# Soltanilara/av-aloha

Hardware: AMD Instinct MI355X
Metric: env-steps/sec (whole node) at 4096 parallel envs, SlotInsertion-3Arms (higher is better)
Workload: dtype f32

## Files before the change

av_aloha_amd/csrc/avsim_api.hip:

```cpp
#include <hip/hip_runtime.h>

#include <cmath>
#include <cstdarg>
#include <cstdio>
#include <cstdlib>
#include <cstring>
#include <memory>
#include <string>
#include <thread>
#include <vector>

#include "../../include/avsim.h"
#include "avsim_episode.hip.h"
#include "avsim_ik.hip.h"
#include "avsim_jpeg.hip.h"
#include "avsim_model.h"
#include "avsim_phys.hip.h"
#include "avsim_render.hip.h"
#include "avsim_vis.hip.h"

using namespace avs;

static thread_local std::string g_create_error;

// ... 352 lines not shown
        h->nq = b.scalar("nq"); h->nv = b.scalar("nv"); h->nu = b.scalar("nu");
        h->task_id = b.scalar("task_id"); h->num_arms = b.scalar("num_arms");
        h->nj = h->num_arms == 3 ? 21 : 14;
        static const int mx[5] = {4, 4, 5, 3, 4};
        h->max_reward = mx[h->task_id];
        h->obj_qadr = b.i("objects_qposadr");
        h->nobj = (int)h->obj_qadr.size();
        h->obs_qadr = b.i("obs_qposadr");
        h->qpos_home = b.f("qpos_home");
        h->ctrl_home = b.f("ctrl_home");
        fill_ik(b, h->ik);
        std::string perr;
        if (!h->phys.init(b, num_envs, h->f64, perr)) { g_create_error = perr; return AVSIM_EMODEL; }
        h->render.build(b, num_envs);
        h->vis.keep_instances(b);
    } catch (const std::exception& ex) {
        g_create_error = std::string("avsim_create: ") + ex.what();
        return AVSIM_EMODEL;
    }
    e = hipStreamCreateWithFlags(&h->stream, hipStreamNonBlocking);
    if (e != hipSuccess) { g_create_error = std::string("hipStreamCreate: ") + hipGetErrorString(e); return AVSIM_EHIP; }
    h->own_stream = true;
    for (auto& ev : h->ev) (void)hipEventCreate(&ev);
    size_t N = num_envs, r = h->rsz();
    if (hipMalloc(&h->d_qpos, N * h->nq * r) != hipSuccess || hipMalloc(&h->d_qvel, N * h->nv * r) != hipSuccess ||
        hipMalloc(&h->d_ctrl, N * h->nu * r) != hipSuccess || hipMalloc(&h->d_warm, N * h->nv * r) != hipSuccess ||
        hipMalloc((void**)&h->d_latch, N * sizeof(int)) != hipSuccess) {
        g_create_error = "avsim_create: hipMalloc of the state arrays failed";
        avsim_destroy(h.release());
        return AVSIM_EHIP;
// ... 751 lines not shown
```

av_aloha_amd/csrc/avsim_phys.hip.h:

```cpp
#pragma once
#include <hip/hip_runtime.h>

#include <string>
#include <vector>

#include "avsim_collide.hip.h"
#include "avsim_math.hip.h"
#include "avsim_model.h"

namespace avs {

enum { J_FREE = 0, J_BALL = 1, J_SLIDE = 2, J_HINGE = 3 };
enum { R_EQ = 0, R_FLOSS = 1, R_LIMIT = 2, R_CONTACT = 3 };
constexpr int TREE_W = 8;
constexpr int ROW_W = 2 * TREE_W;
constexpr int ROW_S = ROW_W;
constexpr int RS_S = 9;
constexpr int CAND_MAX = 256;
constexpr int PROF_W = 26;
constexpr int ANC_MAX = 64;
constexpr int NEAR_MAX = 512;

template <typename real>
struct DevModel {
    int nq, nv, nu, nbody, njnt, ngeom, npair, ntree, neq, nfloss, nlimited, nment, task_id, nj, msize;
    real timestep, gravity[3], impratio, grip_lo, grip_hi;
    int noslip_iters;
    int noslip_trees;
    int qcqp_tridiag;
    int newton_early_exit;
    int newton_component;
    int noslip_per_tree;
    int solver, newton_iters;
    real newton_tol, nscale;
    real ls_tolerance;
    int ls_iterations;
// ... 55 lines not shown
    GLB_PTR(const int) eq_qpos1;
    GLB_PTR(const int) eq_qpos2;
    GLB_PTR(const real) eq_polycoef;
    GLB_PTR(const real) eq_solref;
    GLB_PTR(const real) eq_solimp;
    GLB_PTR(const real) qpos0;
    GLB_PTR(const real) qpos_home;
    int nobj;
    GLB_PTR(const int) obj_qadr;
    const double* obj_reset;
    GLB_PTR(const int) geom_type;
    GLB_PTR(const int) geom_body;
    GLB_PTR(const int) geom_hull;
    GLB_PTR(const int) geom_class;
    GLB_PTR(const int) geom_static;
    GLB_PTR(const real) geom_pos;
    GLB_PTR(const real) geom_mat;
    GLB_PTR(const real) geom_size;
    GLB_PTR(const real) geom_cpos;
    GLB_PTR(const real) geom_rbound;
    GLB_PTR(const real) geom_xpos0;
    GLB_PTR(const real) geom_xmat0;
    GLB_PTR(const real) geom_cen0;
    GLB_PTR(const real) geom_aabb0;
    GLB_PTR(const real) geom_lbox;
    GLB_PTR(const real) hull_vert;
    int hull_ovf;
    GLB_PTR(const int) pair_geom;
    GLB_PTR(const int) pair_condim;
    GLB_PTR(const real) pair_friction;
    GLB_PTR(const real) pair_solref;
    GLB_PTR(const real) pair_solimp;
    GLB_PTR(const real) pair_margin;
    GLB_PTR(const real) pair_gap;
    real* rJ_glob;
    real* rB_glob;
    real* gA_glob;
    int* near_glob;
    int* cand_glob;
    real* gref_glob;
    real* bxo_glob;
    GLB_PTR(const int) obs_qposadr;
    GLB_PTR(const real) obs_offset;
    GLB_PTR(const real) obs_scale;
};

struct MOff {
    int nreal, nint;
    int body_parent;
// ... 1930 lines not shown
        {
            const int t = lane >> 3, i = lane & 7;
            const bool mine = t < ka->m.ntree && i < tree_dofnum_()[t];
            const int k = mine ? tree_dofadr_()[t] + i : 0;
            const real x = tree_solve(r + ka->lay.L, mine ? as[k] : real(0));
            GSYNC();
            if (mine) as[k] = x;
        }
        GSYNC();
    }

    __device__ void load_shape(int g, Shape<real>& s) {
        LDS_BASES();
        real *xpos = r + ka->lay.xpos, *xmat = r + ka->lay.xmat, *gcen = r + ka->lay.gcen;
        s.type = geom_type_()[g];
        for (int k = 0; k < 3; k++) s.size[k] = ka->m.geom_size[3 * g + k];
        s.hull = ka->m.hull_vert;
        s.hbase = ka->m.geom_hull[2 * g];
        s.hR = ka->m.geom_hull[2 * g + 1];
        s.hovf = ka->m.hull_ovf;
        s.nh = 0;
        for (int k = 0; k < 3; k++) { s.lc[k] = ka->m.geom_lbox[6 * g + k]; s.lh[k] = ka->m.geom_lbox[6 * g + 3 + k]; }
        if (geom_static_()[g]) {
            for (int k = 0; k < 3; k++) { s.pos[k] = ka->m.geom_xpos0[3 * g + k]; s.center[k] = ka->m.geom_cen0[3 * g + k]; }
            for (int k = 0; k < 9; k++) s.mat[k] = ka->m.geom_xmat0[9 * g + k];
        } else {
            int b = geom_body_()[g];
            real gp[3] = {ka->m.geom_pos[3 * g], ka->m.geom_pos[3 * g + 1], ka->m.geom_pos[3 * g + 2]}, t3[3];
            mulmat(xmat + 9 * b, gp, t3);
            for (int k = 0; k < 3; k++) { s.pos[k] = xpos[3 * b + k] + t3[k]; s.center[k] = gcen[3 * g + k]; }
            const real* Rb = xmat + 9 * b;
            GLB_PTR(const real) Rg = ka->m.geom_mat + 9 * g;
            for (int i = 0; i < 3; i++)
                for (int j = 0; j < 3; j++) s.mat[3 * i + j] = Rb[3 * i] * Rg[j] + Rb[3 * i + 1] * Rg[3 + j] + Rb[3 * i + 2] * Rg[6 + j];
        }
    }

    __device__ AVS_OUTLINE_0 static void multi_perturb(KPtr<real> ka_, real* r_, int* i_, int lane_, int grp_, const real* lr_, const int* li_, int env_,
                                                                   int pga, int pgb, int src, int pert) {
        Env e(ka_, r_, i_, lane_, grp_, lr_, li_);
        e.env = env_;
        LDS_PTR(real) os = (LDS_PTR(real))(e.r + e.ka->lay.scr + SLOT_W * src);
        const real p0[3] = {os[SLOT_P], os[SLOT_P + 1], os[SLOT_P + 2]}, n0[3] = {os[SLOT_N], os[SLOT_N + 1], os[SLOT_N + 2]};
        Shape<real> a, b;
        e.load_shape(pga, a);
        e.load_shape(pgb, b);
        real dk = real(1e30), pk[3] = {0, 0, 0};
        if (!mpr_perturbed(a, b, p0, n0, pert, &dk, pk)) dk = real(1e30);
        os[1 + pert] = dk;
        for (int c = 0; c < 3; c++) os[SLOT_P + 3 * (1 + pert) + c] = pk[c];
    }

    __device__ AVS_OUTLINE void collide() {
        Env e(*this);
        e.collide_i();
        diverged = e.diverged; nit_sum = e.nit_sum; nit_max = e.nit_max; t_broad = e.t_broad; t_narrow = e.t_narrow;
    }
    __device__ __attribute__((always_inline)) void collide_i() {
        PHASE_BEGIN();
        real* gcen = r + ka->lay.gcen;
        int* misc = ii + ka->lay.misc;
        GLB_PTR(int) cand = cand_();
        int ncand = 0;
        long long tb0 = __builtin_readcyclecounter();
        const real skin = real(0.03);
        GLB_PTR(real) gref = gref_();
        GLB_PTR(int) nearl = near_();
        auto pair_hit = [&](int p, real pad) -> bool {
            int g1 = ka->m.pair_geom[2 * p], g2 = ka->m.pair_geom[2 * p + 1];
            bool s1 = geom_static_()[g1], s2 = geom_static_()[g2];
            real mg = ka->m.pair_margin[p] + pad;
            if (s1 || s2) {
                int gs = s1 ? g1 : g2, gd = s1 ? g2 : g1;
                real rd = geom_rbound_()[gd] + mg, d2 = 0;
                for (int k = 0; k < 3; k++) {
                    real c = gcen[3 * gd + k], lo = ka->m.geom_aabb0[6 * gs + k], hi = ka->m.geom_aabb0[6 * gs + 3 + k];
                    real e = c < lo ? lo - c : (c > hi ? c - hi : real(0));
                    d2 += e * e;
                }
                return !(d2 > rd * rd);
            }
            real d[3], rr = geom_rbound_()[g1] + geom_rbound_()[g2] + mg;
            sub3(gcen + 3 * g2, gcen + 3 * g1, d);
            return !(dot3(d, d) > rr * rr);
        };
        bool moved = false;
        if (misc[7]) {
            for (int g = lane; g < ka->m.ngeom; g += G)
                if (!geom_static_()[g]) {
                    const real d[3] = {gcen[3 * g] - gref[3 * g], gcen[3 * g + 1] - gref[3 * g + 1], gcen[3 * g + 2] - gref[3 * g + 2]};
                    moved |= dot3(d, d) > real(0.25) * skin * skin;
                }
        }
        bool rebuild = !misc[7] || __any(moved);
        int nnear = misc[6];
        if (rebuild) {
            nnear = 0;
            for (int base = 0; base < ka->m.npair; base += G) {
                int p = base + lane;
                bool hit = p < ka->m.npair && pair_hit(p, skin);
                int tot, rk = group_rank<G>(hit, grp, lane, &tot);
                if (hit && nnear + rk < NEAR_MAX) nearl[nnear + rk] = p;
                nnear += tot;
            }
            for (int i = lane; i < 3 * ka->m.ngeom; i += G) gref[i] = gcen[i];
            if (lane == 0) { misc[6] = nnear < NEAR_MAX ? nnear : NEAR_MAX; misc[7] = nnear <= NEAR_MAX; if (nnear > NEAR_MAX) misc[2] |= 8; }
            GSYNC();
        }
        if (nnear <= NEAR_MAX) {
            for (int base = 0; base < nnear; base += G) {
                int i = base + lane, p = i < nnear ? nearl[i] : 0;
                bool hit = i < nnear && pair_hit(p, real(0));
                int tot, rk = group_rank<G>(hit, grp, lane, &tot);
                if (hit && ncand + rk < CAND_MAX) cand[ncand + rk] = p;
                if (ncand + tot > CAND_MAX && lane == 0) misc[2] |= 4;
                ncand = ncand + tot < CAND_MAX ? ncand + tot : CAND_MAX;
            }
        } else {
            for (int base = 0; base < ka->m.npair; base += G) {
                int p = base + lane;
                bool hit = p < ka->m.npair && pair_hit(p, real(0));
                int tot, rk = group_rank<G>(hit, grp, lane, &tot);
                if (hit && ncand + rk < CAND_MAX) cand[ncand + rk] = p;
                if (ncand + tot > CAND_MAX && lane == 0) misc[2] |= 4;
                ncand = ncand + tot < CAND_MAX ? ncand + tot : CAND_MAX;
            }
        }
        if (lane == 0) misc[3] = ncand;
        GSYNC();
        long long tb1 = __builtin_readcyclecounter();
        t_broad += tb1 - tb0;
        real *cdist = r + ka->lay.cdist, *cpos = r + ka->lay.cpos, *cnrm = r + ka->lay.cnrm;
        int* cpair = ii + ka->lay.cpair;
        int ncon = 0, ovf = 0;
        int* mlist = ii + ka->lay.cand;
        GLB_PTR(real) bxo = bxo_();
        for (int base = 0; base < ncand; base += G) {
            const int ci = base + lane;
            int n = 0, p = 0, nn = 0;
            LDS_PTR(real) scr = (LDS_PTR(real))(r + ka->lay.scr + SLOT_W * lane);
            const bool valid = ci < ncand;
            if (valid) p = cand[ci];
            const int ga = ka->m.pair_geom[2 * p], gb = ka->m.pair_geom[2 * p + 1];
            const int tya = geom_type_()[ga], tyb = geom_type_()[gb];
            const bool isbox = valid && tya == G_BOX && tyb == G_BOX;
            const long long tn0_ = profiling ? __builtin_readcyclecounter() : 0;
            {
                bool boxlive = false;
                if (isbox) {
                    Shape<real> a, b;
                    load_shape(ga, a);
                    load_shape(gb, b);
                    boxlive = !boxes_separated(a, b);
                }
                int nbox, rk = group_rank<G>(boxlive, grp, lane, &nbox);
                const int row = lane >> 4;
                for (int b0 = 0; b0 < nbox; b0 += 4) {
                    int src = 0;
// ... 47 lines not shown
                            const real dk = scr[k];
                            const real pk[3] = {scr[SLOT_P + 3 * k], scr[SLOT_P + 3 * k + 1], scr[SLOT_P + 3 * k + 2]};
                            if (dk < real(1e29) && multiccd_distinct(pk, scr + SLOT_P, kept, tol)) {
                                scr[kept] = dk;
                                for (int c = 0; c < 3; c++) scr[SLOT_P + 3 * kept + c] = pk[c];
                                kept++;
                            }
                        }
                        nn = kept;
                    }
                }
            }
            int keepmask = 0;
            GLB_PTR(const real) ov = bxo + BOX_OVF_W * lane;
            if (valid) {
                real mg = ka->m.pair_margin[p];
                for (int k = 0; k < nn; k++)
                    if ((isbox && k >= BOX_SLOTC ? ov[4 * (k - BOX_SLOTC)] : scr[k]) < mg) { keepmask |= 1 << k; n++; }
            }
            int off = 0, tot = 0;
            for (int j = 1; j <= BOX_MAXC; j++) {
                int tj, rj = group_rank<G>(n >= j, grp, lane, &tj);
                if (tj == 0) break;
                off += rj;
                tot += tj;
            }
            int w = 0;
            for (int k = 0; k < BOX_MAXC; k++)
                if ((keepmask >> k) & 1) {
                    int c = ncon + off + w;
                    w++;
// ... 53 lines not shown
            }
            int t1, t2, r1 = group_rank<G>(lo, grp, lane, &t1), r2 = group_rank<G>(hi, grp, lane, &t2);
            int pos = nefc + r1 + r2;
            if (lo && pos < ka->lay.maxefc) rmeta[pos] = R_LIMIT | (j << 2) | (0 << 12);
            if (hi && pos + lo < ka->lay.maxefc) rmeta[pos + lo] = R_LIMIT | (j << 2) | (1 << 12);
            nefc += t1 + t2;
        }
        int ovf = 0;
        if (nefc > ka->lay.maxefc) { nefc = ka->lay.maxefc; ovf = 1; }
        if (lane == 0) misc[4] = nefc;
        const int nlead0 = nefc;
        int cend = nefc;
        for (int base = 0; base < ncon; base += G) {
            int c = base + lane, dim = 0;
            if (c < ncon) {
                int p = cpair[c];
                if (cdist[c] < ka->m.pair_margin[p] - ka->m.pair_gap[p]) dim = ka->m.pair_condim[p];
            }
            int off = 0, tot = 0;
            for (int j = 1; j <= 6; j++) {
                int tj, rj = group_rank<G>(dim >= j, grp, lane, &tj);
                off += rj;
                tot += tj;
            }
            int myend = 0;
            if (c < ncon) {
                int first = nefc + off;
                if (dim > 0 && first + dim <= ka->lay.maxefc) {
                    cefc[c] = first | (dim << 16);
                    myend = first + dim;
                    for (int s = 0; s < dim; s++) rmeta[first + s] = R_CONTACT | (c << 2) | (s << 12) | (dim << 20);
                } else {
// ... 51 lines not shown
                j1 = d - tree_dofadr_()[tA]; v1 = 1;
                for (int k = 0; k < 2; k++) solref[k] = ka->m.dof_solref[2 * d + k];
                for (int k = 0; k < 5; k++) solimp[k] = ka->m.dof_solimp[5 * d + k];
            } else if (LEAD && type == R_LIMIT) {
                int j = id, d = jnt_dofadr_()[j];
                real q = qpos[jnt_qposadr_()[j]];
                tA = dof_tree_()[d];
                pos = sub == 0 ? q - jnt_range_()[2 * j] : jnt_range_()[2 * j + 1] - q;
                margin = jnt_margin_()[j];
                diag0 = dof_invweight0_()[d];
                j1 = d - tree_dofadr_()[tA]; v1 = sub == 0 ? real(1) : real(-1);
                for (int k = 0; k < 2; k++) solref[k] = ka->m.jnt_solref[2 * j + k];
                for (int k = 0; k < 5; k++) solimp[k] = ka->m.jnt_solimp[5 * j + k];
            } else if (!LEAD) {
                int c = id, p = cpair[c];
                int g1 = ka->m.pair_geom[2 * p], g2 = ka->m.pair_geom[2 * p + 1], b1 = geom_body_()[g1], b2 = geom_body_()[g2];
                int t1 = body_tree_()[b1], t2 = body_tree_()[b2];
                tA = t1 >= 0 ? t1 : t2;
                tB = (t1 >= 0 && t2 >= 0 && t2 != t1) ? t2 : -1;
                real n[3] = {cnrm[3 * c], cnrm[3 * c + 1], cnrm[3 * c + 2]}, t1v[3], t2v[3], cp[3] = {cpos[3 * c], cpos[3 * c + 1], cpos[3 * c + 2]};
                make_frame(n, t1v, t2v);
                const int sm = sub % 3;
                real ax[3];
#pragma unroll
                for (int q = 0; q < 3; q++) ax[q] = sm == 0 ? n[q] : (sm == 1 ? t1v[q] : t2v[q]);
                const bool rot = sub >= 3;
                real cx[3], Wa[3], Wl[3];
                cross3(cp, ax, cx);
#pragma unroll
                for (int q = 0; q < 3; q++) { Wa[q] = rot ? ax[q] : cx[q]; Wl[q] = rot ? real(0) : ax[q]; }
                const int mA = (t1 == tA ? bmask[b1] : 0), pA = (t2 == tA ? bmask[b2] : 0);
// ... 2 lines not shown
#pragma unroll
                for (int k = 0; k < TREE_W; k++) {
                    const real* ca = cdofp + 6 * (aA + k < nvm ? aA + k : nvm);
                    const real ea = Wa[0] * ca[0] + Wa[1] * ca[1] + Wa[2] * ca[2] + Wl[0] * ca[3] + Wl[1] * ca[4] + Wl[2] * ca[5];
                    J[k] = real(((pA >> k) & 1) - ((mA >> k) & 1)) * ea;
                }
                if (tB >= 0) {
#pragma unroll
                    for (int k = 0; k < TREE_W; k++) {
                        const real* cb = cdofp + 6 * (aB + k < nvm ? aB + k : nvm);
                        const real eb = Wa[0] * cb[0] + Wa[1] * cb[1] + Wa[2] * cb[2] + Wl[0] * cb[3] + Wl[1] * cb[4] + Wl[2] * cb[5];
                        J[TREE_W + k] = real(((pB >> k) & 1) - ((mB >> k) & 1)) * eb;
                    }
                }
                pos = sub == 0 ? cdist[c] : real(0);
                margin = ka->m.pair_margin[p] - ka->m.pair_gap[p];
                diag0 = body_invweight0_()[2 * b1] + body_invweight0_()[2 * b2];
                for (int k = 0; k < 2; k++) solref[k] = ka->m.pair_solref[2 * p + k];
                for (int k = 0; k < 5; k++) solimp[k] = ka->m.pair_solimp[5 * p + k];
            }
            (void)valid;
            const int j2c = j2 >= 0 ? j2 : (j1 >= 0 ? j1 : 0), j1c = j1 >= 0 ? j1 : 0;
            const real v2c = j2 >= 0 ? v2 : real(0);
            if (LEAD) {
#pragma unroll
                for (int k = 0; k < TREE_W; k++) J[k] += (k == j1 ? v1 : real(0)) + (k == j2 ? v2 : real(0));
            }
            real dmax = tclamp(solimp[1], real(0.0001), real(0.9999));
            real tc = tmax(solref[0], 2 * ka->m.timestep), dr = solref[1];
            real K = real(1) / tmax(real(1e-15), dmax * dmax * tc * tc * dr * dr), Bd = real(2) / tmax(real(1e-15), dmax * tc);
            real imp, R;
            const real imp_row = impedance(solimp, (!LEAD && sub > 0) ? cdist[id] : pos, margin);
            if (!LEAD && sub > 0) {
                int c = id, p = cpair[c];
                real imp0 = imp_row;
                real R0 = tmax(real(1e-15), (1 - imp0) * diag0 / imp0);
                real R1 = R0 / tmax(real(1e-15), ka->m.impratio);
                real mu0 = ka->m.pair_friction[5 * p], mur = ka->m.pair_friction[5 * p + sub - 1];
                R = sub == 1 ? R1 : R1 * mu0 * mu0 / tmax(real(1e-15), mur * mur);
                imp = imp0;
                K = 0;
                floss = mur;
            } else {
                imp = imp_row;
                R = tmax(real(1e-15), (1 - imp) * diag0 / imp);
            }
            real vel = 0;
            if (LEAD) {
                const int a0 = tadr[tA];
                vel = v1 * qvel[a0 + j1c] + v2c * qvel[a0 + j2c];
            } else {
                const int a0 = tadr[tA], b0 = tadr[tB >= 0 ? tB : tA];
#pragma unroll
// ... 89 lines not shown
        for (int i = lane; i < nlead0; i += G) fill(i, BoolTag<true>{});
        ROWPROBE(1);
        for (int i = nlead0 + lane; i < nefc; i += G) fill(i, BoolTag<false>{});
        GSYNC();
        ROWPROBE(2);
        int* gI = ii + ka->lay.gI;
        GLB_PTR(real) gA = coup_();
        const int nlead = misc[4];
        int ngrp = 0;
        for (int base = 0; base < nefc; base += G) {
            int i = base + lane;
            bool head = false;
            int cnt = 0, isc = 0;
            if (i < nefc) {
                if (i < nlead) { head = (i % GRP_MAX) == 0; cnt = nlead - i < GRP_MAX ? nlead - i : GRP_MAX; }
                else { int meta = rmeta[i]; head = ((meta >> 12) & 255) == 0; cnt = ka->m.pair_condim[cpair[(meta >> 2) & 1023]]; isc = 1; }
            }
            int tot, rk = group_rank<G>(head, grp, lane, &tot);
            if (head && ngrp + rk < ka->lay.maxgrp) gI[ngrp + rk] = i | (cnt << 16) | (isc << 24);
            ngrp += tot;
        }
        if (ngrp > ka->lay.maxgrp) ngrp = ka->lay.maxgrp;
        if (lane == 0) misc[5] = ngrp;
        GSYNC();
        ROWPROBE(3);
        const int nlg = (nlead + GRP_MAX - 1) / GRP_MAX;
        const int per_c = newton ? 10 : 15, nl15 = lead_slim ? 0 : nlg * 15, nitem = ngrp <= nlg ? (lead_slim ? 0 : ngrp * 15) : nl15 + (ngrp - nlg) * per_c;
        for (int w = lane; w < nitem; w += G) {
            int g, e, rr = 1, ss;
            if (w < nl15 || !newton) {
                g = w / 15; e = w - 15 * g;
// ... 121 lines not shown
                done_ = noslip_trees<real>((LDS_PTR(real))rowS, (LDS_PTR(const int))rowI, (LDS_PTR(const int))cefc, (GLB_PTR(const real))rJ, (LDS_PTR(real))qacc,
                                           (LDS_PTR(const int))(ii + ka->lay.gI), (GLB_PTR(const real))coup_(), ncon, nefc, ka->m.noslip_iters, real(1e-6) / ka->m.nscale, NL_ARGS(noslip_lead()));
            if (__builtin_amdgcn_readfirstlane(done_) == 2)
                done_ = noslip_trees2<real>((LDS_PTR(real))rowS, (LDS_PTR(const int))rowI, (LDS_PTR(const int))cefc, (GLB_PTR(const real))rJ, (GLB_PTR(const real))rowsB_(), (LDS_PTR(real))qacc,
                                            (LDS_PTR(const int))(ii + ka->lay.gI), (GLB_PTR(const real))coup_(), ncon, nefc, ka->m.noslip_iters, real(1e-6) / ka->m.nscale, NL_ARGS(noslip_lead()));
            if (__builtin_amdgcn_readfirstlane(done_) != 1 && lane == 0) misc[8] = 1;
            if (__builtin_amdgcn_readfirstlane(done_) != 1)
            pgs_groups<real>((LDS_PTR(real))rowS, (LDS_PTR(const int))rowI, (GLB_PTR(const real))rJ, (GLB_PTR(const real))rowsB_(), (LDS_PTR(real))qacc,
                             (LDS_PTR(const int))(ii + ka->lay.gI), (GLB_PTR(const real))coup_(), misc[5], 0, ka->m.noslip_iters, real(1e-6) / ka->m.nscale, NL_ARGS(noslip_lead()));
            if (profiling && lane == 0) (ii + ka->lay.nprof)[6] += (int)(__builtin_readcyclecounter() - tn0);
        } else {
        for (int c = lane; c < ncon; c += G) {
            int first = cefc[c];
            if (first < 0) continue;
            first &= 0xffff;
            int dim = ka->m.pair_condim[(ii + ka->lay.cpair)[c]];
            real fn = rowS[RS_S * first + 6], s2 = 0;
            for (int s = 1; s < dim; s++) { real t = rowS[RS_S * (first + s) + 6] * rowS[RS_S * (first + s) + 7]; s2 += t * t; }
            if (s2 > fn * fn) { real sc = fn / sqrt(s2); for (int s = 1; s < dim; s++) rowS[RS_S * (first + s) + 6] *= sc; }
        }
        GSYNC();
        jt_force(fcon, nefc);
        for (int k = lane; k < ka->m.nv; k += G) {
            int t = dof_tree_()[k], a0 = tree_dofadr_()[t], kk = k - a0, n = tree_dofnum_()[t];
            real s = as[k];
            for (int j = 0; j < n; j++) s += Minv[64 * t + 8 * kk + j] * fcon[a0 + j];
            qacc[k] = s;
        }
        GSYNC();
        static_assert(G == 64, "the solver maps one env to one wavefront");
        pgs_groups<real>((LDS_PTR(real))rowS, (LDS_PTR(const int))rowI, (GLB_PTR(const real))rJ, (GLB_PTR(const real))rowsB_(), (LDS_PTR(real))qacc,
// ... 75 lines not shown
            } else {
                qpos[qa] += h * qvel[da];
            }
        }
        GSYNC();
    }

    __device__ int reward(int* latch) {
        PHASE_BEGIN();
        int *misc = ii + ka->lay.misc, *cpair = ii + ka->lay.cpair;
        int ncon = misc[0];
        int f = 0;
        const int t = ka->m.task_id;
        for (int c = lane; c < ncon; c += G) {
            int p = cpair[c];
            f |= reward_pair_flags(ka->m.geom_class[ka->m.pair_geom[2 * p]], ka->m.geom_class[ka->m.pair_geom[2 * p + 1]], t);
        }
        for (int o = 1; o < G; o <<= 1) f |= __shfl_xor(f, o, G);
        return reward_from_flags(f, t, latch);
    }
};

#ifndef AVSIM_PHYS_MAXW
#define AVSIM_PHYS_MAXW 8
#endif
template <typename real, int G, int MAXW, bool RETRY>
#ifndef AVSIM_PHYS_ATTR
#ifdef AVSIM_TU_F64
#define AVSIM_PHYS_ATTR
#else
#define AVSIM_PHYS_ATTR __attribute__((amdgpu_waves_per_eu(2)))
// ... 174 lines not shown
        for (int i = lane; i < ka->m.nj; i += G) o_agent[(size_t)env * ka->m.nj + i] = ((double)r[ka->lay.qpos + ka->m.obs_qposadr[i]] - (double)ka->m.obs_offset[i]) * (double)ka->m.obs_scale[i];
    int ncon = ii[ka->lay.misc + 0];
    if (want_reward) {
        int latch = g_latch[env];
        int rw = E.reward(&latch);
        if (lane == 0) {
            g_latch[env] = latch;
            if (o_reward) o_reward[env] = rw;
            if (o_success) o_success[env] = (rw == max_reward);
        }
    }
    if (export_contacts)
    {
    const int expcon = RETRY ? ka->lay.expcon : ka->lay.maxcon;
    for (int c = lane; c < expcon; c += G) {
        int p = c < ncon ? ii[ka->lay.cpair + c] : -1;
        o_cpairs[((size_t)env * expcon + c) * 2] = p >= 0 ? ka->m.pair_geom[2 * p] : -1;
        o_cpairs[((size_t)env * expcon + c) * 2 + 1] = p >= 0 ? ka->m.pair_geom[2 * p + 1] : -1;
        o_cdist[(size_t)env * expcon + c] = c < ncon ? (double)r[ka->lay.cdist + c] : 0.0;
    }
    }
    if (lane == 0 && o_cost && nsub > 0) o_cost[env] = (int)((__builtin_readcyclecounter() - t_launch) >> 6);
    if (lane == 0 && !o_xpose) {
        o_ncon[env] = ncon;
        bool bad = E.diverged != 0;
        for (int i = 0; i < ka->m.nq; i++) bad |= !(fabs(r[ka->lay.qpos + i]) < real(1e6));
        o_diag[4 * env] = ncon; o_diag[4 * env + 1] = nefc_last; o_diag[4 * env + 2] = ii[ka->lay.misc + 2]; o_diag[4 * env + 3] = (bad ? 1 : 0) | ((ii[ka->lay.misc + 3] & 0xff) << 8) | ((E.nit_sum & 0xfff) << 16) | ((E.nit_max < 15 ? E.nit_max : 15) << 28);
    }
    GSYNC();
    if (RETRY && big && pass1) {
        lds_put(&pair_want[pr], 0);
    }
  }
// ... 228 lines not shown
                    double ex[3] = {gsize[3 * g], gsize[3 * g + 1], gsize[3 * g + 2]};
                    if (gtype[g] == G_SPHERE) ex[1] = ex[2] = ex[0];
                    if (gtype[g] == G_CYLINDER) { ex[2] = ex[1]; ex[1] = ex[0]; }
                    for (int c = 0; c < 8; c++) for (int k = 0; k < 3; k++) pts.push_back(((c >> k) & 1) ? ex[k] : -ex[k]);
                }
                for (int k = 0; k < 3; k++) { gaabb[6 * g + k] = 1e30; gaabb[6 * g + 3 + k] = -1e30; }
                for (size_t v = 0; v < pts.size() / 3; v++)
                    for (int i = 0; i < 3; i++) {
                        double w = gx0[3 * g + i] + gm0[9 * g + 3 * i] * pts[3 * v] + gm0[9 * g + 3 * i + 1] * pts[3 * v + 1] + gm0[9 * g + 3 * i + 2] * pts[3 * v + 2];
                        if (w < gaabb[6 * g + i]) gaabb[6 * g + i] = w;
                        if (w > gaabb[6 * g + 3 + i]) gaabb[6 * g + 3 + i] = w;
                    }
            }
        }
        m.geom_type = up(I("geom_type")); moff.geom_type = (int)img_int.size(); { auto v_ = I("geom_type"); img_int.insert(img_int.end(), v_.begin(), v_.end()); } m.geom_body = up(gbody); moff.geom_body = (int)img_int.size(); { auto v_ = gbody; img_int.insert(img_int.end(), v_.begin(), v_.end()); } m.geom_hull = up(I("geom_ctab")); m.geom_class = up(I("geom_class")); m.geom_static = up(gstat); moff.geom_static = (int)img_int.size(); { auto v_ = gstat; img_int.insert(img_int.end(), v_.begin(), v_.end()); }
        m.geom_pos = upr<real>(gpos); m.geom_mat = upr<real>(gmat); m.geom_size = upr<real>(F("geom_size")); m.geom_cpos = upr<real>(gcp); moff.geom_cpos = (int)img_real.size(); { auto v_ = gcp; img_real.insert(img_real.end(), v_.begin(), v_.end()); }
        m.geom_rbound = upr<real>(F("geom_rbound")); moff.geom_rbound = (int)img_real.size(); { auto v_ = F("geom_rbound"); img_real.insert(img_real.end(), v_.begin(), v_.end()); } m.geom_xpos0 = upr<real>(gx0); m.geom_xmat0 = upr<real>(gm0); m.geom_cen0 = upr<real>(gc0); m.geom_aabb0 = upr<real>(gaabb); m.geom_lbox = upr<real>(glbox);
        {
            auto ctab = I("geom_ctab"), cells = I("chull_cells"), cand = I("chull_cand");
            const size_t ncell = cells.size();
            std::vector<double> tab(32 * ncell, 0.0), ovf;
            std::vector<char> done(ncell, 0);
            for (int g = 0; g < ng; g++) {
                if (gtype[g] != G_MESH) continue;
                const int cb = ctab[2 * g], R = ctab[2 * g + 1], adr = ghull[2 * g];
                for (int c = 0; c < 6 * R * R; c++) {
                    if (done[cb + c]) continue;
                    done[cb + c] = 1;
                    const int rec = cells[cb + c], off = rec >> 8, cnt = rec & 255;
                    if (cnt < 1) throw std::runtime_error("support table: empty cell");
                    double* o = &tab[32 * (size_t)(cb + c)];
                    for (int k = 0; k < 8; k++) {
// ... 6 lines not shown
                    o[7] = (double)(ovf.size() / 4);
                    for (int k = 8; k < cnt; k++) {
                        const int v = cand[off + k];
                        if (v < 0 || v >= ghull[2 * g + 1]) throw std::runtime_error("support table: candidate index outside its hull");
                        for (int q = 0; q < 3; q++) ovf.push_back(hv[3 * (size_t)(adr + v) + q]);
                        ovf.push_back((double)v);
                    }
                }
            }
            if (ovf.size() / 4 >= (1u << 24)) throw std::runtime_error("support table: overflow part too large");
            m.hull_ovf = (int)(tab.size() / 4);
            tab.insert(tab.end(), ovf.begin(), ovf.end());
            if (tab.empty()) tab.assign(4, 0.0);
            m.hull_vert = upr<real>(tab);
        }
        m.pair_geom = up(I("pair_geom")); m.pair_condim = up(I("pair_condim"));
        m.pair_friction = upr<real>(F("pair_friction")); m.pair_solref = upr<real>(F("pair_solref")); m.pair_solimp = upr<real>(F("pair_solimp"));
        m.pair_margin = upr<real>(F("pair_margin")); m.pair_gap = upr<real>(F("pair_gap"));
        m.obs_qposadr = up(I("obs_qposadr")); m.obs_offset = upr<real>(F("obs_offset")); m.obs_scale = upr<real>(F("obs_scale"));
        while (img_real.size() % 4) img_real.push_back(0.0);
        while (img_int.size() % 4) img_int.push_back(0);
        moff.nreal = (int)img_real.size();
        moff.nint = (int)img_int.size();
        d_img_real = (void*)upr<real>(img_real);
        d_img_int = up(img_int);
    }

    void make_layout(int nq, int nv, int nu, int nb, int ng, int msize, int ntree) {
        if (maxcon1 > maxcon) maxcon1 = maxcon;
        if (maxefc1 > maxefc) maxefc1 = maxefc;
        make_layout_of(lay, maxcon1, maxefc1, nq, nv, nu, nb, ng, msize, ntree);
        make_layout_of(lay2, maxcon, maxefc, nq, nv, nu, nb, ng, msize, ntree);
    }
// ... 81 lines not shown
            maxefc = cap_efc[b.scalar("task_id")];
            maxcon = cap_con[b.scalar("task_id")];
            maxefc1 = cap_efc1[b.scalar("task_id")];
            maxcon1 = cap_con1[b.scalar("task_id")];
            dims[0] = b.scalar("nq"); dims[1] = b.scalar("nv"); dims[2] = b.scalar("nu"); dims[3] = b.scalar("nbody"); dims[4] = b.scalar("ngeom"); dims[5] = ms; dims[6] = b.scalar("ntree");
            make_layout(dims[0], dims[1], dims[2], dims[3], dims[4], dims[5], dims[6]);
            d_qpos_home = up(b.f("qpos_home"));
            d_ctrl_home = up(b.f("ctrl_home"));
            d_obj_qadr = up(b.i("objects_qposadr"));
            d_ncon = up(std::vector<int>((size_t)N, 0));
            d_diag = up(std::vector<int>((size_t)N * 4, 0));
            d_cost = up(std::vector<int>((size_t)N, 0));
            d_order = up(std::vector<int>((size_t)N, 0));
            d_retry = up(std::vector<int>(2 * (size_t)N + 2, 0));
            alloc_contacts();
        } catch (const std::exception& e) {
            err = std::string("physics init: ") + e.what();
            return false;
        }
        return true;
    }
    void destroy() {
        for (void* p : allocs) (void)hipFree(p);
        allocs.clear();
        if (d_cpairs) (void)hipFree(d_cpairs);
        if (d_cdist) (void)hipFree(d_cdist);
        if (d_rows) (void)hipFree(d_rows);
        if (d_coup) (void)hipFree(d_coup);
        if (d_near) (void)hipFree(d_near);
        if (d_gref) (void)hipFree(d_gref);
// ... 2 lines not shown
    bool set_option(const char* name, double v) {
        std::string n(name);
        kargs_dirty = true;
        if (n == "pgs_iters") { pgs_iters = (int)v; return true; }
        if (n == "solver") { if (v != 0 && v != 1) return false; mf.solver = md.solver = (int)v; return true; }
        if (n == "newton_iters") { if (v < 1 || v > 100) return false; mf.newton_iters = md.newton_iters = (int)v; return true; }
        if (n == "newton_tol") { if (v < 0) return false; mf.newton_tol = (float)v; md.newton_tol = v; return true; }
        if (n == "ls_tolerance") { if (!(v > 0) || v >= 1) return false; mf.ls_tolerance = (float)v; md.ls_tolerance = v; return true; }
        if (n == "ls_iterations") { if (v < 1 || v > 1000) return false; mf.ls_iterations = md.ls_iterations = (int)v; return true; }
        if (n == "export_contacts") { export_contacts = v != 0; return true; }
        if (n == "num_joints") { if (v != 14 && v != 21) return false; mf.nj = md.nj = (int)v; return true; }
        if (n == "order_envs") { order_envs = v != 0; return true; }
        if (n == "pair_waves") { pair_waves = v != 0; return true; }
        if (n == "qcqp_tridiag") { mf.qcqp_tridiag = md.qcqp_tridiag = v < 0 ? 0 : (v > 2 ? 2 : (int)v); return true; }
        if (n == "noslip_per_tree") { mf.noslip_per_tree = md.noslip_per_tree = v != 0; return true; }
        if (n == "noslip_trees") { mf.noslip_trees = md.noslip_trees = v != 0; return true; }
        if (n == "newton_component") { mf.newton_component = md.newton_component = v != 0; return true; }
        if (n == "newton_early_exit") { mf.newton_early_exit = md.newton_early_exit = v != 0; return true; }
        if (n == "persist_blocks") { int x = (int)v; if (x >= 1 && x <= 64) { persist_over = x; return true; } return false; }
        if (n == "waves_per_block") { int x = (int)v; if (x >= 0 && x <= AVSIM_PHYS_MAXW) { wpb_override = x; return true; } return false; }
        if (n == "profile_phases") {
            if (v != 0 && !d_prof) d_prof = up(std::vector<long long>((size_t)N * PROF_W, 0));
            if (v == 0) d_prof = nullptr;
            return true;
        }
        if (n == "maxefc" || n == "maxcon" || n == "maxefc_first" || n == "maxcon_first") {
            int x = (int)v;
            if (x < 16 || x > 1000) return false;
            (void)hipDeviceSynchronize();
            if (n == "maxefc") maxefc = maxefc1 = x; else if (n == "maxcon") maxcon = maxcon1 = x;
// ... 105 lines not shown
```

Measured before the change: 977,600.

## Pack pair records into words with deduplicated class tables and per-geom records

Contact pairs are now stored as packed 32-bit words (geom1, geom2, parameter class, pair index), and the per-pair friction/solref/solimp/margin/gap/condim values are deduplicated into a small class table. Per-geom static data is merged into one 24-wide record that is loaded with vector loads. When LDS has room, the candidate pair list goes in LDS instead of global memory. The aim is fewer scattered global loads in the collision and constraint-setup paths, at the cost of hard limits on geom, class and pair counts, plus a new error path.

```diff
diff --git a/av_aloha_amd/csrc/avsim_api.hip b/av_aloha_amd/csrc/avsim_api.hip
--- a/av_aloha_amd/csrc/avsim_api.hip
+++ b/av_aloha_amd/csrc/avsim_api.hip
@@ -390,6 +390,9 @@
         if (!h->phys.init(b, num_envs, h->f64, perr)) { g_create_error = perr; return AVSIM_EMODEL; }
         h->render.build(b, num_envs);
         h->vis.keep_instances(b);
+    } catch (const avs::pair_limit_error& ex) {
+        g_create_error = std::string("avsim_create: ") + ex.what();
+        return AVSIM_EINVAL;
     } catch (const std::exception& ex) {
         g_create_error = std::string("avsim_create: ") + ex.what();
         return AVSIM_EMODEL;
diff --git a/av_aloha_amd/csrc/avsim_pairs.h b/av_aloha_amd/csrc/avsim_pairs.h
--- /dev/null
+++ b/av_aloha_amd/csrc/avsim_pairs.h
@@ -0,0 +1,73 @@
+#pragma once
+#include <cstdint>
+#include <cstring>
+#include <stdexcept>
+#include <string>
+#include <vector>
+
+#if defined(__HIPCC__) || defined(__CUDACC__)
+#define AVS_PAIRS_HD __host__ __device__ inline
+#else
+#define AVS_PAIRS_HD inline
+#endif
+
+namespace avs {
+
+constexpr int PW_GEOM_BITS = 7, PW_CLASS_BITS = 6, PW_PAIR_BITS = 12;
+constexpr int PW_MAX_GEOMS = 1 << PW_GEOM_BITS, PW_MAX_CLASSES = 1 << PW_CLASS_BITS, PW_MAX_PAIRS = 1 << PW_PAIR_BITS;
+static_assert(2 * PW_GEOM_BITS + PW_CLASS_BITS + PW_PAIR_BITS == 32, "the pair word is 32 bits");
+
+constexpr int PC_W = 16;
+constexpr int PC_MARGIN = 0, PC_GAP = 1, PC_SOLREF = 2, PC_SOLIMP = 4, PC_FRICTION = 9, PC_CONDIM = 14;
+
+AVS_PAIRS_HD uint32_t pw_pack(int g1, int g2, int cls, int pair) {
+    return (uint32_t)g1 | ((uint32_t)g2 << PW_GEOM_BITS) | ((uint32_t)cls << (2 * PW_GEOM_BITS)) | ((uint32_t)pair << (2 * PW_GEOM_BITS + PW_CLASS_BITS));
+}
+AVS_PAIRS_HD int pw_geom1(int w) { return (int)((uint32_t)w & (PW_MAX_GEOMS - 1)); }
+AVS_PAIRS_HD int pw_geom2(int w) { return (int)(((uint32_t)w >> PW_GEOM_BITS) & (PW_MAX_GEOMS - 1)); }
+AVS_PAIRS_HD int pw_class(int w) { return (int)(((uint32_t)w >> (2 * PW_GEOM_BITS)) & (PW_MAX_CLASSES - 1)); }
+AVS_PAIRS_HD int pw_pair(int w) { return (int)((uint32_t)w >> (2 * PW_GEOM_BITS + PW_CLASS_BITS)); }
+
+struct pair_limit_error : std::runtime_error {
+    using std::runtime_error::runtime_error;
+};
+
+template <typename real>
+struct PairTables {
+    std::vector<int> word;
+    std::vector<real> cls;
+    int ncls = 0;
+};
+
+template <typename real>
+PairTables<real> build_pair_tables(int npair, int ngeom, const int* pair_geom, const int* condim, const double* friction, const double* solref,
+                                   const double* solimp, const double* margin, const double* gap) {
+    if (ngeom > PW_MAX_GEOMS) throw pair_limit_error("pair records: " + std::to_string(ngeom) + " geoms, the pair word holds geom ids below " + std::to_string(PW_MAX_GEOMS));
+    if (npair > PW_MAX_PAIRS) throw pair_limit_error("pair records: " + std::to_string(npair) + " contact pairs, the pair word holds pair indices below " + std::to_string(PW_MAX_PAIRS));
+    PairTables<real> t;
+    t.word.resize(npair > 0 ? npair : 0);
+    for (int p = 0; p < npair; p++) {
+        const int g1 = pair_geom[2 * p], g2 = pair_geom[2 * p + 1];
+        if (g1 < 0 || g2 < 0 || g1 >= ngeom || g2 >= ngeom) throw pair_limit_error("pair records: pair " + std::to_string(p) + " names a geom outside 0.." + std::to_string(ngeom - 1));
+        if (condim[p] < 1 || condim[p] > 6) throw pair_limit_error("pair records: pair " + std::to_string(p) + " has condim " + std::to_string(condim[p]) + " outside 1..6");
+        real row[PC_W];
+        for (int k = 0; k < PC_W; k++) row[k] = real(0);
+        row[PC_MARGIN] = (real)margin[p];
+        row[PC_GAP] = (real)gap[p];
+        for (int k = 0; k < 2; k++) row[PC_SOLREF + k] = (real)solref[2 * p + k];
+        for (int k = 0; k < 5; k++) row[PC_SOLIMP + k] = (real)solimp[5 * p + k];
+        for (int k = 0; k < 5; k++) row[PC_FRICTION + k] = (real)friction[5 * p + k];
+        row[PC_CONDIM] = (real)condim[p];
+        int c = 0;
+        while (c < t.ncls && std::memcmp(&t.cls[(size_t)PC_W * c], row, sizeof(row)) != 0) c++;
+        if (c == t.ncls) {
+            if (t.ncls == PW_MAX_CLASSES) throw pair_limit_error("pair records: more than " + std::to_string(PW_MAX_CLASSES) + " distinct pair parameter rows (condim, friction, solref, solimp, margin, gap)");
+            t.cls.insert(t.cls.end(), row, row + PC_W);
+            t.ncls++;
+        }
+        t.word[p] = (int)pw_pack(g1, g2, c, p);
+    }
+    return t;
+}
+
+}
diff --git a/av_aloha_amd/csrc/avsim_phys.hip.h b/av_aloha_amd/csrc/avsim_phys.hip.h
--- a/av_aloha_amd/csrc/avsim_phys.hip.h
+++ b/av_aloha_amd/csrc/avsim_phys.hip.h
@@ -7,6 +7,7 @@
 #include "avsim_collide.hip.h"
 #include "avsim_math.hip.h"
 #include "avsim_model.h"
+#include "avsim_pairs.h"
 
 namespace avs {
 
@@ -20,6 +21,8 @@
 constexpr int PROF_W = 26;
 constexpr int ANC_MAX = 64;
 constexpr int NEAR_MAX = 512;
+
+constexpr int GR_W = 24, GR_SIZE = 0, GR_LC = 3, GR_LH = 6, GR_POS = 9, GR_MAT = 12, GR_CEN = 21;
 
 template <typename real>
 struct DevModel {
@@ -105,25 +108,15 @@
     GLB_PTR(const int) geom_hull;
     GLB_PTR(const int) geom_class;
     GLB_PTR(const int) geom_static;
-    GLB_PTR(const real) geom_pos;
-    GLB_PTR(const real) geom_mat;
-    GLB_PTR(const real) geom_size;
+    GLB_PTR(const real) geom_rec;
     GLB_PTR(const real) geom_cpos;
     GLB_PTR(const real) geom_rbound;
-    GLB_PTR(const real) geom_xpos0;
-    GLB_PTR(const real) geom_xmat0;
-    GLB_PTR(const real) geom_cen0;
     GLB_PTR(const real) geom_aabb0;
-    GLB_PTR(const real) geom_lbox;
     GLB_PTR(const real) hull_vert;
     int hull_ovf;
-    GLB_PTR(const int) pair_geom;
-    GLB_PTR(const int) pair_condim;
-    GLB_PTR(const real) pair_friction;
-    GLB_PTR(const real) pair_solref;
-    GLB_PTR(const real) pair_solimp;
-    GLB_PTR(const real) pair_margin;
-    GLB_PTR(const real) pair_gap;
+    GLB_PTR(const int) pair_word;
+    GLB_PTR(const real) pair_class;
+    int near_always;
     real* rJ_glob;
     real* rB_glob;
     real* gA_glob;
@@ -2084,23 +2077,30 @@
         LDS_BASES();
         real *xpos = r + ka->lay.xpos, *xmat = r + ka->lay.xmat, *gcen = r + ka->lay.gcen;
         s.type = geom_type_()[g];
-        for (int k = 0; k < 3; k++) s.size[k] = ka->m.geom_size[3 * g + k];
+        real rec[GR_W];
+        {
+            typedef real real4 __attribute__((ext_vector_type(4)));
+            GLB_PTR(const real4) q = (GLB_PTR(const real4))(ka->m.geom_rec + GR_W * g);
+#pragma unroll
+            for (int i = 0; i < GR_W / 4; i++) { const real4 v = q[i]; rec[4 * i] = v.x; rec[4 * i + 1] = v.y; rec[4 * i + 2] = v.z; rec[4 * i + 3] = v.w; }
+        }
+        for (int k = 0; k < 3; k++) s.size[k] = rec[GR_SIZE + k];
         s.hull = ka->m.hull_vert;
         s.hbase = ka->m.geom_hull[2 * g];
         s.hR = ka->m.geom_hull[2 * g + 1];
         s.hovf = ka->m.hull_ovf;
         s.nh = 0;
-        for (int k = 0; k < 3; k++) { s.lc[k] = ka->m.geom_lbox[6 * g + k]; s.lh[k] = ka->m.geom_lbox[6 * g + 3 + k]; }
+        for (int k = 0; k < 3; k++) { s.lc[k] = rec[GR_LC + k]; s.lh[k] = rec[GR_LH + k]; }
         if (geom_static_()[g]) {
-            for (int k = 0; k < 3; k++) { s.pos[k] = ka->m.geom_xpos0[3 * g + k]; s.center[k] = ka->m.geom_cen0[3 * g + k]; }
-            for (int k = 0; k < 9; k++) s.mat[k] = ka->m.geom_xmat0[9 * g + k];
+            for (int k = 0; k < 3; k++) { s.pos[k] = rec[GR_POS + k]; s.center[k] = rec[GR_CEN + k]; }
+            for (int k = 0; k < 9; k++) s.mat[k] = rec[GR_MAT + k];
         } else {
             int b = geom_body_()[g];
-            real gp[3] = {ka->m.geom_pos[3 * g], ka->m.geom_pos[3 * g + 1], ka->m.geom_pos[3 * g + 2]}, t3[3];
+            real gp[3] = {rec[GR_POS], rec[GR_POS + 1], rec[GR_POS + 2]}, t3[3];
             mulmat(xmat + 9 * b, gp, t3);
             for (int k = 0; k < 3; k++) { s.pos[k] = xpos[3 * b + k] + t3[k]; s.center[k] = gcen[3 * g + k]; }
             const real* Rb = xmat + 9 * b;
-            GLB_PTR(const real) Rg = ka->m.geom_mat + 9 * g;
+            const real* Rg = rec + GR_MAT;
             for (int i = 0; i < 3; i++)
                 for (int j = 0; j < 3; j++) s.mat[3 * i + j] = Rb[3 * i] * Rg[j] + Rb[3 * i + 1] * Rg[3 + j] + Rb[3 * i + 2] * Rg[6 + j];
         }
@@ -2130,16 +2130,20 @@
         PHASE_BEGIN();
         real* gcen = r + ka->lay.gcen;
         int* misc = ii + ka->lay.misc;
-        GLB_PTR(int) cand = cand_();
+        const bool cand_lds = 2 * ka->lay.maxefc >= CAND_MAX;
+        GLB_PTR(int) candg = cand_();
+        int* const candl = ii + ka->lay.rmeta;
+        auto cand_put = [&](int i, int w) { if (cand_lds) candl[i] = w; else candg[i] = w; };
         int ncand = 0;
         long long tb0 = __builtin_readcyclecounter();
         const real skin = real(0.03);
         GLB_PTR(real) gref = gref_();
         GLB_PTR(int) nearl = near_();
-        auto pair_hit = [&](int p, real pad) -> bool {
-            int g1 = ka->m.pair_geom[2 * p], g2 = ka->m.pair_geom[2 * p + 1];
+        GLB_PTR(const real) pcls = ka->m.pair_class;
+        auto pair_hit = [&](int w, real pad) -> bool {
+            int g1 = pw_geom1(w), g2 = pw_geom2(w);
             bool s1 = geom_static_()[g1], s2 = geom_static_()[g2];
-            real mg = ka->m.pair_margin[p] + pad;
+            real mg = pcls[PC_W * pw_class(w) + PC_MARGIN] + pad;
             if (s1 || s2) {
                 int gs = s1 ? g1 : g2, gd = s1 ? g2 : g1;
                 real rd = geom_rbound_()[gd] + mg, d2 = 0;
@@ -2162,15 +2166,16 @@
                     moved |= dot3(d, d) > real(0.25) * skin * skin;
                 }
         }
-        bool rebuild = !misc[7] || __any(moved);
+        bool rebuild = !misc[7] || ka->m.near_always || __any(moved);
         int nnear = misc[6];
         if (rebuild) {
             nnear = 0;
             for (int base = 0; base < ka->m.npair; base += G) {
                 int p = base + lane;
-                bool hit = p < ka->m.npair && pair_hit(p, skin);
+                const int w = p < ka->m.npair ? ka->m.pair_word[p] : 0;
+                bool hit = p < ka->m.npair && pair_hit(w, skin);
                 int tot, rk = group_rank<G>(hit, grp, lane, &tot);
-                if (hit && nnear + rk < NEAR_MAX) nearl[nnear + rk] = p;
+                if (hit && nnear + rk < NEAR_MAX) nearl[nnear + rk] = w;
                 nnear += tot;
             }
             for (int i = lane; i < 3 * ka->m.ngeom; i += G) gref[i] = gcen[i];
@@ -2179,19 +2184,20 @@
         }
         if (nnear <= NEAR_MAX) {
             for (int base = 0; base < nnear; base += G) {
-                int i = base + lane, p = i < nnear ? nearl[i] : 0;
-                bool hit = i < nnear && pair_hit(p, real(0));
+                int i = base + lane, w = i < nnear ? nearl[i] : 0;
+                bool hit = i < nnear && pair_hit(w, real(0));
                 int tot, rk = group_rank<G>(hit, grp, lane, &tot);
-                if (hit && ncand + rk < CAND_MAX) cand[ncand + rk] = p;
+                if (hit && ncand + rk < CAND_MAX) cand_put(ncand + rk, w);
                 if (ncand + tot > CAND_MAX && lane == 0) misc[2] |= 4;
                 ncand = ncand + tot < CAND_MAX ? ncand + tot : CAND_MAX;
             }
         } else {
             for (int base = 0; base < ka->m.npair; base += G) {
                 int p = base + lane;
-                bool hit = p < ka->m.npair && pair_hit(p, real(0));
+                const int w = p < ka->m.npair ? ka->m.pair_word[p] : 0;
+                bool hit = p < ka->m.npair && pair_hit(w, real(0));
                 int tot, rk = group_rank<G>(hit, grp, lane, &tot);
-                if (hit && ncand + rk < CAND_MAX) cand[ncand + rk] = p;
+                if (hit && ncand + rk < CAND_MAX) cand_put(ncand + rk, w);
                 if (ncand + tot > CAND_MAX && lane == 0) misc[2] |= 4;
                 ncand = ncand + tot < CAND_MAX ? ncand + tot : CAND_MAX;
             }
@@ -2210,8 +2216,8 @@
             int n = 0, p = 0, nn = 0;
             LDS_PTR(real) scr = (LDS_PTR(real))(r + ka->lay.scr + SLOT_W * lane);
             const bool valid = ci < ncand;
-            if (valid) p = cand[ci];
-            const int ga = ka->m.pair_geom[2 * p], gb = ka->m.pair_geom[2 * p + 1];
+            if (valid) p = cand_lds ? candl[ci] : candg[ci];
+            const int ga = pw_geom1(p), gb = pw_geom2(p);
             const int tya = geom_type_()[ga], tyb = geom_type_()[gb];
             const bool isbox = valid && tya == G_BOX && tyb == G_BOX;
             const long long tn0_ = profiling ? __builtin_readcyclecounter() : 0;
@@ -2289,7 +2295,7 @@
             int keepmask = 0;
             GLB_PTR(const real) ov = bxo + BOX_OVF_W * lane;
             if (valid) {
-                real mg = ka->m.pair_margin[p];
+                real mg = pcls[PC_W * pw_class(p) + PC_MARGIN];
                 for (int k = 0; k < nn; k++)
                     if ((isbox && k >= BOX_SLOTC ? ov[4 * (k - BOX_SLOTC)] : scr[k]) < mg) { keepmask |= 1 << k; n++; }
             }
@@ -2373,8 +2379,8 @@
         for (int base = 0; base < ncon; base += G) {
             int c = base + lane, dim = 0;
             if (c < ncon) {
-                int p = cpair[c];
-                if (cdist[c] < ka->m.pair_margin[p] - ka->m.pair_gap[p]) dim = ka->m.pair_condim[p];
+                GLB_PTR(const real) pc = ka->m.pair_class + PC_W * pw_class(cpair[c]);
+                if (cdist[c] < pc[PC_MARGIN] - pc[PC_GAP]) dim = (int)pc[PC_CONDIM];
             }
             int off = 0, tot = 0;
             for (int j = 1; j <= 6; j++) {
@@ -2456,7 +2462,8 @@
                 for (int k = 0; k < 5; k++) solimp[k] = ka->m.jnt_solimp[5 * j + k];
             } else if (!LEAD) {
                 int c = id, p = cpair[c];
-                int g1 = ka->m.pair_geom[2 * p], g2 = ka->m.pair_geom[2 * p + 1], b1 = geom_body_()[g1], b2 = geom_body_()[g2];
+                GLB_PTR(const real) pc = ka->m.pair_class + PC_W * pw_class(p);
+                int g1 = pw_geom1(p), g2 = pw_geom2(p), b1 = geom_body_()[g1], b2 = geom_body_()[g2];
                 int t1 = body_tree_()[b1], t2 = body_tree_()[b2];
                 tA = t1 >= 0 ? t1 : t2;
                 tB = (t1 >= 0 && t2 >= 0 && t2 != t1) ? t2 : -1;
@@ -2489,10 +2496,10 @@
                     }
                 }
                 pos = sub == 0 ? cdist[c] : real(0);
-                margin = ka->m.pair_margin[p] - ka->m.pair_gap[p];
+                margin = pc[PC_MARGIN] - pc[PC_GAP];
                 diag0 = body_invweight0_()[2 * b1] + body_invweight0_()[2 * b2];
-                for (int k = 0; k < 2; k++) solref[k] = ka->m.pair_solref[2 * p + k];
-                for (int k = 0; k < 5; k++) solimp[k] = ka->m.pair_solimp[5 * p + k];
+                for (int k = 0; k < 2; k++) solref[k] = pc[PC_SOLREF + k];
+                for (int k = 0; k < 5; k++) solimp[k] = pc[PC_SOLIMP + k];
             }
             (void)valid;
             const int j2c = j2 >= 0 ? j2 : (j1 >= 0 ? j1 : 0), j1c = j1 >= 0 ? j1 : 0;
@@ -2507,11 +2514,11 @@
             real imp, R;
             const real imp_row = impedance(solimp, (!LEAD && sub > 0) ? cdist[id] : pos, margin);
             if (!LEAD && sub > 0) {
-                int c = id, p = cpair[c];
+                GLB_PTR(const real) pc = ka->m.pair_class + PC_W * pw_class(cpair[id]);
                 real imp0 = imp_row;
                 real R0 = tmax(real(1e-15), (1 - imp0) * diag0 / imp0);
                 real R1 = R0 / tmax(real(1e-15), ka->m.impratio);
-                real mu0 = ka->m.pair_friction[5 * p], mur = ka->m.pair_friction[5 * p + sub - 1];
+                real mu0 = pc[PC_FRICTION], mur = pc[PC_FRICTION + sub - 1];
                 R = sub == 1 ? R1 : R1 * mu0 * mu0 / tmax(real(1e-15), mur * mur);
                 imp = imp0;
                 K = 0;
@@ -2631,7 +2638,7 @@
             int cnt = 0, isc = 0;
             if (i < nefc) {
                 if (i < nlead) { head = (i % GRP_MAX) == 0; cnt = nlead - i < GRP_MAX ? nlead - i : GRP_MAX; }
-                else { int meta = rmeta[i]; head = ((meta >> 12) & 255) == 0; cnt = ka->m.pair_condim[cpair[(meta >> 2) & 1023]]; isc = 1; }
+                else { int meta = rmeta[i]; head = ((meta >> 12) & 255) == 0; cnt = (int)ka->m.pair_class[PC_W * pw_class(cpair[(meta >> 2) & 1023]) + PC_CONDIM]; isc = 1; }
             }
             int tot, rk = group_rank<G>(head, grp, lane, &tot);
             if (head && ngrp + rk < ka->lay.maxgrp) gI[ngrp + rk] = i | (cnt << 16) | (isc << 24);
@@ -2783,7 +2790,7 @@
             int first = cefc[c];
             if (first < 0) continue;
             first &= 0xffff;
-            int dim = ka->m.pair_condim[(ii + ka->lay.cpair)[c]];
+            int dim = (int)ka->m.pair_class[PC_W * pw_class((ii + ka->lay.cpair)[c]) + PC_CONDIM];
             real fn = rowS[RS_S * first + 6], s2 = 0;
             for (int s = 1; s < dim; s++) { real t = rowS[RS_S * (first + s) + 6] * rowS[RS_S * (first + s) + 7]; s2 += t * t; }
             if (s2 > fn * fn) { real sc = fn / sqrt(s2); for (int s = 1; s < dim; s++) rowS[RS_S * (first + s) + 6] *= sc; }
@@ -2889,7 +2896,7 @@
         const int t = ka->m.task_id;
         for (int c = lane; c < ncon; c += G) {
             int p = cpair[c];
-            f |= reward_pair_flags(ka->m.geom_class[ka->m.pair_geom[2 * p]], ka->m.geom_class[ka->m.pair_geom[2 * p + 1]], t);
+            f |= reward_pair_flags(ka->m.geom_class[pw_geom1(p)], ka->m.geom_class[pw_geom2(p)], t);
         }
         for (int o = 1; o < G; o <<= 1) f |= __shfl_xor(f, o, G);
         return reward_from_flags(f, t, latch);
@@ -3094,9 +3101,9 @@
     {
     const int expcon = RETRY ? ka->lay.expcon : ka->lay.maxcon;
     for (int c = lane; c < expcon; c += G) {
-        int p = c < ncon ? ii[ka->lay.cpair + c] : -1;
-        o_cpairs[((size_t)env * expcon + c) * 2] = p >= 0 ? ka->m.pair_geom[2 * p] : -1;
-        o_cpairs[((size_t)env * expcon + c) * 2 + 1] = p >= 0 ? ka->m.pair_geom[2 * p + 1] : -1;
+        const int p = c < ncon ? ii[ka->lay.cpair + c] : 0;
+        o_cpairs[((size_t)env * expcon + c) * 2] = c < ncon ? pw_geom1(p) : -1;
+        o_cpairs[((size_t)env * expcon + c) * 2 + 1] = c < ncon ? pw_geom2(p) : -1;
         o_cdist[(size_t)env * expcon + c] = c < ncon ? (double)r[ka->lay.cdist + c] : 0.0;
     }
     }
@@ -3355,8 +3362,21 @@
             }
         }
         m.geom_type = up(I("geom_type")); moff.geom_type = (int)img_int.size(); { auto v_ = I("geom_type"); img_int.insert(img_int.end(), v_.begin(), v_.end()); } m.geom_body = up(gbody); moff.geom_body = (int)img_int.size(); { auto v_ = gbody; img_int.insert(img_int.end(), v_.begin(), v_.end()); } m.geom_hull = up(I("geom_ctab")); m.geom_class = up(I("geom_class")); m.geom_static = up(gstat); moff.geom_static = (int)img_int.size(); { auto v_ = gstat; img_int.insert(img_int.end(), v_.begin(), v_.end()); }
-        m.geom_pos = upr<real>(gpos); m.geom_mat = upr<real>(gmat); m.geom_size = upr<real>(F("geom_size")); m.geom_cpos = upr<real>(gcp); moff.geom_cpos = (int)img_real.size(); { auto v_ = gcp; img_real.insert(img_real.end(), v_.begin(), v_.end()); }
-        m.geom_rbound = upr<real>(F("geom_rbound")); moff.geom_rbound = (int)img_real.size(); { auto v_ = F("geom_rbound"); img_real.insert(img_real.end(), v_.begin(), v_.end()); } m.geom_xpos0 = upr<real>(gx0); m.geom_xmat0 = upr<real>(gm0); m.geom_cen0 = upr<real>(gc0); m.geom_aabb0 = upr<real>(gaabb); m.geom_lbox = upr<real>(glbox);
+        m.geom_cpos = upr<real>(gcp); moff.geom_cpos = (int)img_real.size(); { auto v_ = gcp; img_real.insert(img_real.end(), v_.begin(), v_.end()); }
+        m.geom_rbound = upr<real>(F("geom_rbound")); moff.geom_rbound = (int)img_real.size(); { auto v_ = F("geom_rbound"); img_real.insert(img_real.end(), v_.begin(), v_.end()); } m.geom_aabb0 = upr<real>(gaabb);
+        {
+            std::vector<double> grec((size_t)GR_W * ng, 0.0);
+            for (int g = 0; g < ng; g++) {
+                double* o = &grec[(size_t)GR_W * g];
+                for (int k = 0; k < 3; k++) {
+                    o[GR_SIZE + k] = gsize[3 * g + k]; o[GR_LC + k] = glbox[6 * g + k]; o[GR_LH + k] = glbox[6 * g + 3 + k];
+                    o[GR_POS + k] = gstat[g] ? gx0[3 * g + k] : gpos[3 * g + k];
+                    o[GR_CEN + k] = gstat[g] ? gc0[3 * g + k] : 0.0;
+                }
+                for (int k = 0; k < 9; k++) o[GR_MAT + k] = gstat[g] ? gm0[9 * g + k] : gmat[9 * g + k];
+            }
+            m.geom_rec = upr<real>(grec);
+        }
         {
             auto ctab = I("geom_ctab"), cells = I("chull_cells"), cand = I("chull_cand");
             const size_t ncell = cells.size();
@@ -3393,9 +3413,15 @@
             if (tab.empty()) tab.assign(4, 0.0);
             m.hull_vert = upr<real>(tab);
         }
-        m.pair_geom = up(I("pair_geom")); m.pair_condim = up(I("pair_condim"));
-        m.pair_friction = upr<real>(F("pair_friction")); m.pair_solref = upr<real>(F("pair_solref")); m.pair_solimp = upr<real>(F("pair_solimp"));
-        m.pair_margin = upr<real>(F("pair_margin")); m.pair_gap = upr<real>(F("pair_gap"));
+        {
+            auto pg = I("pair_geom"), pc = I("pair_condim");
+            auto pf = F("pair_friction"), psr = F("pair_solref"), psi = F("pair_solimp"), pm = F("pair_margin"), pgap = F("pair_gap");
+            const size_t np = (size_t)(m.npair > 0 ? m.npair : 0);
+            if (pg.size() < 2 * np || pc.size() < np || pf.size() < 5 * np || psr.size() < 2 * np || psi.size() < 5 * np || pm.size() < np || pgap.size() < np)
+                throw std::runtime_error("pair arrays shorter than npair");
+            const PairTables<real> pt = build_pair_tables<real>(m.npair, m.ngeom, pg.data(), pc.data(), pf.data(), psr.data(), psi.data(), pm.data(), pgap.data());
+            m.pair_word = up(pt.word); m.pair_class = up(pt.cls); m.near_always = 0;
+        }
         m.obs_qposadr = up(I("obs_qposadr")); m.obs_offset = upr<real>(F("obs_offset")); m.obs_scale = upr<real>(F("obs_scale"));
         while (img_real.size() % 4) img_real.push_back(0.0);
         while (img_int.size() % 4) img_int.push_back(0);
@@ -3507,6 +3533,8 @@
             d_order = up(std::vector<int>((size_t)N, 0));
             d_retry = up(std::vector<int>(2 * (size_t)N + 2, 0));
             alloc_contacts();
+        } catch (const pair_limit_error&) {
+            throw;
         } catch (const std::exception& e) {
             err = std::string("physics init: ") + e.what();
             return false;
@@ -3539,6 +3567,7 @@
         if (n == "pair_waves") { pair_waves = v != 0; return true; }
         if (n == "qcqp_tridiag") { mf.qcqp_tridiag = md.qcqp_tridiag = v < 0 ? 0 : (v > 2 ? 2 : (int)v); return true; }
         if (n == "noslip_per_tree") { mf.noslip_per_tree = md.noslip_per_tree = v != 0; return true; }
+        if (n == "near_rebuild") { mf.near_always = md.near_always = v != 0; return true; }
         if (n == "noslip_trees") { mf.noslip_trees = md.noslip_trees = v != 0; return true; }
         if (n == "newton_component") { mf.newton_component = md.newton_component = v != 0; return true; }
         if (n == "newton_early_exit") { mf.newton_early_exit = md.newton_early_exit = v != 0; return true; }
```

Result: no change. 984,300 (median of 6 runs) (+0.7%).
